# QuantumSavory/LDPCDecoders.jl

Measured on AMD Instinct MI355X. Metric: decoded syndromes/sec (batchdecode!, 50 iters) + achieved HBM GB/s fraction, higher is better.
Workload: dtype f64

## Files before the change

### include/ldpc_mi355x_debug.h

```cpp
#ifndef LDPC_MI355X_DEBUG_H
#define LDPC_MI355X_DEBUG_H

#include "ldpc_mi355x.h"

#ifdef __cplusplus
extern "C" {
#endif

ldpc_status ldpc_debug_team_plan(int64_t nnz, int64_t max_iters, int64_t batch, int32_t cache_mib, int32_t rows_dv,
                                 int32_t out[6]);

ldpc_status ldpc_debug_team_rows(int64_t s, int64_t n, const int64_t *colptr, const int64_t *rowval, int32_t members,
                                 int32_t regs_per_wave, int32_t static_quarters, int32_t *degrees, int32_t *shape,
                                 int32_t *vtab, int32_t *ctab, int32_t *lds_edge, int32_t *reg_edge);

ldpc_status ldpc_debug_team_irr(int64_t s, int64_t n, const int64_t *colptr, const int64_t *rowval, int32_t members,
                                int32_t dc_bucket, int32_t dv_bucket, int32_t *shape, int32_t *ctab2, int32_t *ptab, int32_t *ploc,
                                int32_t *lds_edge, int32_t *posmap);

void *ldpc_debug_process_state(void);
ldpc_status ldpc_debug_adopt_process_state(void *state);

ldpc_status ldpc_debug_div_check(int64_t count, const double *num, const double *den, double *out_core, double *out_ieee);

ldpc_status ldpc_debug_llr_check(int64_t count, const double *odds, double *out_fast, double *out_lib);

#ifdef __cplusplus
}
#endif
#endif
```

### ldpcdecoders.jl_amd/_capi.py

```python
from __future__ import annotations

import ctypes
import os
import subprocess

_HERE = os.path.dirname(os.path.abspath(__file__))
CSRC = os.path.join(_HERE, "csrc")
LIB_PATH = os.environ.get("LDPC_MI355X_LIB") or os.path.join(CSRC, "libldpc_mi355x.so")
EXP_LIB_PATH = os.environ.get("LDPC_MI355X_EXP_LIB") or os.path.join(CSRC, "libldpc_mi355x_exp.so")

LDPC_OK = 0
STATUS_NAMES = {
    0: "LDPC_OK",
    1: "LDPC_ERR_INVALID_ARGUMENT",
    2: "LDPC_ERR_NO_DEVICE",
    3: "LDPC_ERR_HIP",
    4: "LDPC_ERR_OUT_OF_MEMORY",
    5: "LDPC_ERR_UNSUPPORTED",
}

EXPORTED_SYMBOLS = (
    "ldpc_abi_version",
    "ldpc_build_target",
    "ldpc_last_error",
# ... 14 lines not shown
    "ldpc_bp_call_phase_ticks",
    "ldpc_bp_create_multi",
    "ldpc_bp_destroy_multi",
    "ldpc_bp_multi_handle",
    "ldpc_bp_decode_batch_multi",
    "ldpc_bp_decode_batch_multi_bits",
    "ldpc_bp_decode_batch_multi_device",
    "ldpc_bp_multi_last_status",
    "ldpc_bp_multi_get_info",
    "ldpc_osd_create",
    "ldpc_osd_destroy",
    "ldpc_osd_postprocess_batch",
    "ldpc_bpots_create",
    "ldpc_bpots_destroy",
    "ldpc_bpots_kernel",
    "ldpc_bpots_decode_batch",
    "ldpc_bpots_decode_batch_device",
    "ldpc_bitflip_create",
    "ldpc_bitflip_destroy",
    "ldpc_bitflip_kernel",
    "ldpc_bitflip_decode_batch",
    "ldpc_bitflip_decode_batch_device",
)
DEBUG_SYMBOLS = ("ldpc_debug_team_rows", "ldpc_debug_team_plan", "ldpc_debug_div_check", "ldpc_debug_process_state",
                 "ldpc_debug_adopt_process_state", "ldpc_debug_team_irr", "ldpc_debug_llr_check")

MULTI_MAX_DEVICES = 16
EXCHANGE_AUTO, EXCHANGE_COPY, EXCHANGE_RCCL, EXCHANGE_NONE = 0, 1, 2, 3


class LdpcError(RuntimeError):
    def __init__(self, status: int, message: str):
        super().__init__(f"{STATUS_NAMES.get(status, status)}: {message}")
        self.status = status
        self.message = message


class BPInfo(ctypes.Structure):
    _fields_ = [
        ("s", ctypes.c_int64), ("n", ctypes.c_int64), ("nnz", ctypes.c_int64),
        ("max_iters", ctypes.c_int64), ("per", ctypes.c_double),
        ("max_check_degree", ctypes.c_int32), ("max_bit_degree", ctypes.c_int32),
        ("device", ctypes.c_int32), ("tile_syndromes", ctypes.c_int32),
        ("waves_per_tile", ctypes.c_int32), ("resident_tiles", ctypes.c_int32),
        ("workspace_bytes", ctypes.c_int64),
        ("last_kernel", ctypes.c_int32), ("last_team_size", ctypes.c_int32),
        ("last_lds_rows", ctypes.c_int32), ("last_rows_on_chip", ctypes.c_int32), ("reserved_info", ctypes.c_int32 * 2),
# ... 60 lines not shown
    path = EXP_LIB_PATH if experiments else LIB_PATH
    if not os.path.exists(path):
        raise LdpcError(2, f"{path} is not built; run `python -c 'import __graft_entry__ as g; g.build()'` "
                           "or `make -C ldpcdecoders.jl_amd/csrc`. There is no CPU fallback.")
    _one_hip_runtime()
    L = ctypes.CDLL(path)
    vp, i64, i32, f64 = ctypes.c_void_p, ctypes.c_int64, ctypes.c_int32, ctypes.c_double
    L.ldpc_abi_version.restype = i32
    L.ldpc_build_target.restype = ctypes.c_char_p
    L.ldpc_last_error.restype = ctypes.c_char_p
    L.ldpc_device_count.restype = i32
    L.ldpc_trim_memory.restype = i32
    L.ldpc_set_wait_limit_ms.restype = i32
    L.ldpc_set_wait_limit_ms.argtypes = [i64]
    L.ldpc_get_wait_limit_ms.restype = i64
    L.ldpc_debug_team_plan.restype = i32
    L.ldpc_debug_team_plan.argtypes = [i64, i64, i64, i32, i32, ctypes.POINTER(i32 * 6)]
    L.ldpc_debug_div_check.restype = i32
    L.ldpc_debug_div_check.argtypes = [i64, vp, vp, vp, vp]
    L.ldpc_debug_llr_check.restype = i32
    L.ldpc_debug_llr_check.argtypes = [i64, vp, vp, vp]
    L.ldpc_debug_team_irr.restype = i32
    L.ldpc_debug_team_irr.argtypes = [i64, i64, vp, vp, i32, i32, i32, ctypes.POINTER(i32 * 2), vp, vp, vp, vp, vp]
    L.ldpc_debug_team_rows.restype = i32
    L.ldpc_debug_team_rows.argtypes = [i64, i64, vp, vp, i32, i32, i32, ctypes.POINTER(i32 * 2), ctypes.POINTER(i32 * 5), vp, vp, vp, vp]
    L.ldpc_bp_create_multi.restype = i32
    L.ldpc_bp_create_multi.argtypes = [i32, ctypes.POINTER(i32), i32, i64, i64, i64, vp, vp, f64, i64, ctypes.POINTER(BPOptions), ctypes.POINTER(vp)]
    L.ldpc_bp_destroy_multi.restype = i32
    L.ldpc_bp_destroy_multi.argtypes = [vp]
    L.ldpc_bp_multi_handle.restype = vp
    L.ldpc_bp_multi_handle.argtypes = [vp, i32]
    L.ldpc_bp_decode_batch_multi.restype = i32
    L.ldpc_bp_decode_batch_multi.argtypes = [vp, i64, vp, vp, vp, vp, vp]
    L.ldpc_bp_decode_batch_multi_device.restype = i32
    L.ldpc_bp_decode_batch_multi_device.argtypes = [vp, i64, vp, vp, vp, vp, vp, vp]
    L.ldpc_bp_multi_last_status.restype = i32
    L.ldpc_bp_multi_last_status.argtypes = [vp]
    L.ldpc_bp_multi_get_info.restype = i32
    L.ldpc_bp_multi_get_info.argtypes = [vp, ctypes.POINTER(BPMultiInfo)]
    L.ldpc_bp_create.restype = i32
    L.ldpc_bp_create.argtypes = [i64, i64, i64, vp, vp, f64, i64, ctypes.POINTER(BPOptions), ctypes.POINTER(vp)]
    L.ldpc_bp_destroy.restype = i32
    L.ldpc_bp_destroy.argtypes = [vp]
    L.ldpc_bp_get_info.restype = i32
    L.ldpc_bp_get_info.argtypes = [vp, ctypes.POINTER(BPInfo)]
    L.ldpc_bp_decode_batch.restype = i32
# ... 65 lines not shown
```

### ldpcdecoders.jl_amd/csrc/bp_team_kernels.hpp

```cpp
#pragma once
#include "bp_kernels.hpp"

#ifndef LDPC_TEAM_THREADS
#define LDPC_TEAM_THREADS 512
#endif
#ifndef LDPC_TEAM_ROWS_WIDE
#define LDPC_TEAM_ROWS_WIDE 1
#endif
#ifndef LDPC_TEAM_TFORM
#define LDPC_TEAM_TFORM 1
#endif
#ifndef LDPC_TEAM_TEST_DIRECT
#define LDPC_TEAM_TEST_DIRECT 1
#endif
#ifndef LDPC_TEAM_SLEEP
#define LDPC_TEAM_SLEEP 16
#endif

namespace ldpc {

__host__ __device__ constexpr int team_vtab_words(int dv) { return 2 * dv + 1 <= 8 ? 8 : 16; }
__host__ __device__ constexpr bool team_rows_degrees_ok(int dc, int dv) { return dc >= 6 && dc <= 10 && dv >= 3 && dv <= 5; }

template <int DV>
struct TeamVRec {
    int pos[DV], lrow[DV], bit;
};
template <int DV>
__device__ __forceinline__ TeamVRec<DV> team_vrec_load(const int *__restrict__ vt)
{
    static_assert(2 * DV + 1 <= 16, "a position record is at most 16 words");
    typedef int v2i __attribute__((ext_vector_type(2)));
    typedef int v4i __attribute__((ext_vector_type(4)));
    typedef int v8i __attribute__((ext_vector_type(8)));
    constexpr int N = 2 * DV + 1;
    int w[16];
// ... 493 lines not shown
    if (deg == 0) return r;
    return bit_dispatch_flat<1, DV>(Mt, L, loc, deg <= DV ? deg : DV, r);
}

template <int DC, int DV, int THREADS, bool LROWS = false>
constexpr int team_min_waves_per_simd()
{
    if (LROWS && LDPC_TEAM_ROWS_WIDE) return THREADS / 256;
    return min_waves_per_simd<DC, DV, THREADS>() < 4 ? min_waves_per_simd<DC, DV, THREADS>() : 4;
}

template <int DC, int DV, bool WANT_LLR, int THREADS, bool RESUMED, bool LROWS = false, int RR = 0, bool IRR = false>
__global__ void
__launch_bounds__(THREADS, (team_min_waves_per_simd<DC, DV, THREADS, LROWS || IRR>()))
bp_team_kernel(BPParams p, TeamParams tp, const int *__restrict__ row_ptr, const int *__restrict__ edge_bit,
               const int *__restrict__ col_ptr, const int *__restrict__ csc2csr,
               const u64 *__restrict__ synmask, const u64 *__restrict__ nevermask)
{
    static_assert(!(LROWS && RESUMED), "packed tiles are decoded where they lie, all rows in global memory");
    static_assert(RR == 0 || (LROWS && RR == kTeamRegRows), "rows in registers come on top of the rows in LDS");
    static_assert(!IRR || (!LROWS && !RESUMED && RR == 0), "irregular graphs: whole checks in LDS, fresh tiles");
    constexpr int RS = IRR ? 2 : 1;
    constexpr bool kTeamHints = (LDPC_TEAM_LIKELY != 0) && DC <= LDPC_TEAM_LIKELY_DC_MAX;
    constexpr bool TF = LROWS && (LDPC_TEAM_TFORM != 0) && DC <= 8;
    auto rget = [&](const int row) -> double {
        if constexpr (RR > 0) return team_reg_get(row);
        else return 0.0;
    };
    auto rput = [&](const bool on, const int row, const double v) {
        if constexpr (RR > 0) {
            if (on) team_reg_put(row, v);
        }
    };
    extern __shared__ double lds_rows[];
    double *const Lr = lds_rows + (threadIdx.x & 63);
    double *const Ldummy = Lr + (size_t)tp.rows.R * kTile;
    __shared__ int sh_ok;
    __shared__ unsigned int sh_deal[2];
#if !LDPC_TEAM_TEST_DIRECT
    __shared__ u64 sh_mism[THREADS / 64];
#endif
    const int lane = threadIdx.x & 63;
    const int w = __builtin_amdgcn_readfirstlane(threadIdx.x >> 6);
    constexpr int W = THREADS / 64;
    const int s = p.s, n = p.n;
    const double r = p.r;
// ... 178 lines not shown
        const size_t cap_rows = ((size_t)n + 3) & ~(size_t)3;
        unsigned int *const cap32 = (unsigned int *)p.llr + (size_t)tile * cap_rows * kTile;
        double *const cap64 = p.llr + (size_t)tile * cap_rows * kTile;
        auto cap_at = [&](int pos) { return ((size_t)(pos >> 2) * kTile + lane) * 4 + (size_t)(pos & 3); };
        auto capture1 = [&](int pos, double T) {
            if (!cap_on) return;
            if (tp.llr_raw == 4) cap32[cap_at(pos)] = llr_hi32(T);
            else cap64[cap_at(pos)] = T;
        };
        auto capture2 = [&](int pos, double T0, double T1) {
            if (!cap_on) return;
            typedef unsigned int v2u __attribute__((ext_vector_type(2)));
            typedef double v2d __attribute__((ext_vector_type(2)));
            if (tp.llr_raw == 4) *(v2u *)(cap32 + cap_at(pos)) = v2u{llr_hi32(T0), llr_hi32(T1)};
            else *(v2d *)(cap64 + cap_at(pos)) = v2d{T0, T1};
        };
        auto capture4 = [&](int pos, const double (&T)[4]) {
            if (!cap_on) return;
            typedef unsigned int v4u __attribute__((ext_vector_type(4)));
            typedef double v2d __attribute__((ext_vector_type(2)));
            if (tp.llr_raw == 4) *(v4u *)(cap32 + cap_at(pos)) = v4u{llr_hi32(T[0]), llr_hi32(T[1]), llr_hi32(T[2]), llr_hi32(T[3])};
            else { *(v2d *)(cap64 + cap_at(pos)) = v2d{T[0], T[1]}; *(v2d *)(cap64 + cap_at(pos) + 2) = v2d{T[2], T[3]}; }
        };
        auto decide = [&](int pos, int j, double T, bool cap = true) {
            const u64 dec = __ballot(T >= 1.0);
            if (WANT_LLR) {
                if (tp.llr_raw >= 4) { if (cap) capture1(pos, T); }
                else if (tp.llr_raw == 0 && ((active >> lane) & 1ull)) p.llr[((size_t)tile * n + j) * kTile + lane] = llr_of(T, p.llr_exact);
            }
            if (lane == 0) em[j] = dec;
        };
        auto chunk = [&](int c) {
            const int j1 = min(n, (c + 1) * vb);
            int j = c * vb;
            if constexpr (LROWS) {
                constexpr int VT = team_vtab_words(DV);
                if constexpr (kFuseFirst) {
                    if (first) {
                        if (j + 4 == j1) {
                            const int *const vt = csc2csr + (size_t)j * VT;
                            const TeamVRec<DV> A = team_vrec_load<DV>(vt), B = team_vrec_load<DV>(vt + VT), C = team_vrec_load<DV>(vt + 2 * VT),
                                               D = team_vrec_load<DV>(vt + 3 * VT);
                            double T[4];
                            T[0] = bit_update_first<DV, DC, TF>(Mt, Lr, sh_first, syn, lane, A.pos, A.lrow, r, rput);
                            T[1] = bit_update_first<DV, DC, TF>(Mt, Lr, sh_first, syn, lane, B.pos, B.lrow, r, rput);
                            T[2] = bit_update_first<DV, DC, TF>(Mt, Lr, sh_first, syn, lane, C.pos, C.lrow, r, rput);
                            T[3] = bit_update_first<DV, DC, TF>(Mt, Lr, sh_first, syn, lane, D.pos, D.lrow, r, rput);
                            decide(j, A.bit & 0x7fffffff, T[0], false);
                            decide(j + 1, B.bit & 0x7fffffff, T[1], false);
                            decide(j + 2, C.bit & 0x7fffffff, T[2], false);
                            decide(j + 3, D.bit & 0x7fffffff, T[3], false);
                            capture4(j, T);
                            return;
                        }
                        for (; j < j1; ++j) {
                            const TeamVRec<DV> A = team_vrec_load<DV>(csc2csr + (size_t)j * VT);
                            decide(j, A.bit & 0x7fffffff, bit_update_first<DV, DC, TF>(Mt, Lr, sh_first, syn, lane, A.pos, A.lrow, r, rput));
                        }
                        return;
                    }
                }
                auto single = [&](const TeamVRec<DV> &a, const int pa) {
                    if (a.bit >= 0) { decide(pa, a.bit, bit_update_exact_v<DV, TF>(Mt, a.pos, r)); return; }
                    if constexpr (RR > 0) {
                        int lo = a.lrow[0];
#pragma unroll
                        for (int k = 1; k < DV; ++k) lo = min(lo, a.lrow[k]);
                        if (lo <= -2) { decide(pa, a.bit & 0x7fffffff, bit_update_onchip<DV, TF>(Mt, Lr, Ldummy, a.pos, a.lrow, r, rget, rput)); return; }
                    }
                    decide(pa, a.bit & 0x7fffffff, bit_update_mixed<DV, TF>(Mt, Lr, a.pos, a.lrow, r));
                };
                auto two = [&](const TeamVRec<DV> &a, const TeamVRec<DV> &b, const int pa) {
                    int rest = -1;
#pragma unroll
                    for (int k = 1; k < DV; ++k) rest &= a.lrow[k] & b.lrow[k];
                    if ((a.bit | b.bit) >= 0 && tp.pairs) {
                        double T0, T1;
                        bit_update_pair_v<DV, TF>(Mt, a.pos, b.pos, r, T0, T1);
                        decide(pa, a.bit, T0, false);
                        decide(pa + 1, b.bit, T1, false);
                        capture2(pa, T0, T1);
                    } else if (rest == -1 && tp.pairs) {
                        double T0, T1;
                        bit_update_pair_first<DV, TF>(Mt, Lr, a.pos, a.lrow[0], b.pos, b.lrow[0], r, rget, rput, T0, T1);
                        decide(pa, a.bit & 0x7fffffff, T0, false);
                        decide(pa + 1, b.bit & 0x7fffffff, T1, false);
                        capture2(pa, T0, T1);
                    } else {
                        single(a, pa);
                        single(b, pa + 1);
                    }
                };
                int q = j;
                if (LDPC_HOT(q + 4 == j1)) {
                    const int *const vt = csc2csr + (size_t)q * VT;
                    const TeamVRec<DV> A = team_vrec_load<DV>(vt), B = team_vrec_load<DV>(vt + VT), C = team_vrec_load<DV>(vt + 2 * VT),
                                       D = team_vrec_load<DV>(vt + 3 * VT);
                    if (LDPC_HOT(tp.pairs & 2)) {
                        int rest = -1;
#pragma unroll
                        for (int k = 1; k < DV; ++k) rest &= A.lrow[k] & B.lrow[k] & C.lrow[k] & D.lrow[k];
                        if (LDPC_HOT(rest == -1)) {
                            int ps[4][DV];
#pragma unroll
                            for (int k = 0; k < DV; ++k) { ps[0][k] = A.pos[k]; ps[1][k] = B.pos[k]; ps[2][k] = C.pos[k]; ps[3][k] = D.pos[k]; }
                            const int lc[4] = {A.lrow[0], B.lrow[0], C.lrow[0], D.lrow[0]};
                            double T[4];
                            constexpr bool KINDS = LDPC_TEAM_CHUNK_KINDS < 0 ? DV == 3 : LDPC_TEAM_CHUNK_KINDS != 0;
                            const int lmin = min(min(lc[0], lc[1]), min(lc[2], lc[3])), lmax = max(max(lc[0], lc[1]), max(lc[2], lc[3]));
                            if (KINDS && RR > 0 && lmax <= -2) bit_update_multi_first<DV, 4, TF, 2>(Mt, Lr, ps, lc, r, rget, rput, T);
                            else if (KINDS && lmin >= 0) bit_update_multi_first<DV, 4, TF, 1>(Mt, Lr, ps, lc, r, rget, rput, T);
                            else bit_update_multi_first<DV, 4, TF, 0>(Mt, Lr, ps, lc, r, rget, rput, T);
                            decide(q, A.bit & 0x7fffffff, T[0], false);
                            decide(q + 1, B.bit & 0x7fffffff, T[1], false);
                            decide(q + 2, C.bit & 0x7fffffff, T[2], false);
                            decide(q + 3, D.bit & 0x7fffffff, T[3], false);
                            capture4(q, T);
                            return;
                        }
                    }
                    two(A, B, q);
                    two(C, D, q + 2);
                    return;
                }
                for (; q + 1 < j1; q += 2) {
                    const int *const vt = csc2csr + (size_t)q * VT;
                    const TeamVRec<DV> A = team_vrec_load<DV>(vt), B = team_vrec_load<DV>(vt + VT);
                    two(A, B, q);
                }
                for (; q < j1; ++q) single(team_vrec_load<DV>(csc2csr + (size_t)q * VT), q);
                return;
            }
            if constexpr (IRR) {
                for (; j < j1; ++j) {
                    const int c0 = col_ptr[2 * j], bw = col_ptr[2 * j + 1];
                    const int deg = col_ptr[2 * j + 2] - c0;
                    const double T = bw >= 0 ? bit_update<DV>(Mt, csc2csr + c0, deg, r) : bit_update_flat<DV>(Mt, Lr, csc2csr + c0, deg, r);
                    decide(j, bw & 0x7fffffff, T);
                }
// ... 49 lines not shown
        if (lane == 0 && mism) __hip_atomic_fetch_or(&mw[it_t - 1], mism, __ATOMIC_RELAXED, __HIP_MEMORY_SCOPE_AGENT);
#else
        if (lane == 0) sh_mism[w] = mism;
        __syncthreads();
        if (threadIdx.x == 0) {
            u64 part = 0;
#pragma unroll
            for (int q = 0; q < W; ++q) part |= sh_mism[q];
            if (part) __hip_atomic_fetch_or(&mw[it_t - 1], part, __ATOMIC_RELAXED, __HIP_MEMORY_SCOPE_AGENT);
        }
#endif
    };
    auto verdict = [&](const int it_t, const u64 *em_t) {
        const u64 U = uniform64(never | __hip_atomic_load(&mw[it_t - 1], __ATOMIC_RELAXED, __HIP_MEMORY_SCOPE_AGENT));
        const int total = it0 + it_t;
        const u64 newly = active & ~U;
        if ((newly >> lane) & 1ull) { my_iters = total; my_conv = 1; }
        active &= U;
        const u64 spent = __ballot(total >= p.max_iters) & active;
        if ((spent >> lane) & 1ull) { my_iters = total; my_conv = 0; }
        active &= ~spent;
        const u64 stopped = newly | spent;
        if (stopped != 0) {
            for (int j = gw * 64 + lane; j < n; j += GW * 64) fin[j] = (fin[j] & ~stopped) | (em_t[j] & stopped);
        }
        quiet = stopped == 0;
        return total;
    };

    while (active != 0) {
        ++it;
        em = (it & 1) ? em_odd : em_even;
        const u64 t0 = wall_clock64();
        const bool fused = kFuseFirst && it == 1 && !resumed;
        if (!have_check && !fused) check_sweep((it == 1) && !resumed);
        const u64 t1 = wall_clock64();
        if (!(fused && placed) && !team_barrier(ctr, G, rank, ++epoch, tp.fault, tp.ticket, &sh_ok, one_xcd, sh_deal)) return;
        if (!placed) {
            if (threadIdx.x == 0)
                sh_one_xcd = __popc(__hip_atomic_load(xccs, __ATOMIC_RELAXED, __HIP_MEMORY_SCOPE_AGENT)) == 1;
            __syncthreads();
            one_xcd = sh_one_xcd != 0 && !tp.always_release;
            placed = true;
        }
        if (have_check) {
            have_check = false;
            verdict(it - 1, ((it - 1) & 1) ? em_odd : em_even);
// ... 100 lines not shown
```

### ldpcdecoders.jl_amd/csrc/ldpc_mi355x.hip

```cpp
#include "../../include/ldpc_mi355x.h"
#include "../../include/ldpc_mi355x_debug.h"
#define LDPC_AUX_KERNELS 1
#include "bp_kernels.hpp"
#include "bp_lds_kernels.hpp"
#include "bp_node_kernels.hpp"
#include "bp_team_kernels.hpp"
#include "bit_io_kernels.hpp"
#include "pickers.hpp"
#include "host_env.hpp"
#include "host_wait.hpp"

#include <algorithm>
#include <atomic>
#include <chrono>
#include <condition_variable>
#include <cstdio>
#include <cstdlib>
#include <cstring>
#include <memory>
#include <mutex>
#include <new>
#include <string>
#include <thread>
#include <utility>
// ... 384 lines not shown
    int last_rows_on_chip = 0;
    int rows_on_chip = 0;
    size_t ws_budget = 0;
    int blocks_cache[2][17];
    int variant = 0;
    bool node_ok = false;
    bool node_msg_lds = false;
    int node_split_check = 0, node_split_edge = 0;
    int64_t node_max_batch = 0;
    int64_t node_take_max = 0;
    DevBuf node_msg;
    DevBuf team_ws, team_ws_lvl[2];
    std::vector<int> h_csc2csr;
    std::vector<int> h_row_ptr, h_edge_bit, h_col_ptr, h_irr_c2r;
    int irr_G = 0, irr_R = 0, irr_on_chip = 0;
    int irr_dcb = 0;
    DevBuf irr_ctab, irr_ptab, irr_ploc, irr_lds_edge, irr_posmap;
    bool team_rows_on = true;
    int rows_dc = 0, rows_dv = 0;
    int rows_G = 0, rows_R = 0;
    int rows_first_c = 0;
    int rows_regs = 0, rows_static_c = 0, rows_static_v = 0;
    DevBuf rows_ctab, rows_vtab, rows_lds_edge, rows_reg_edge, rows_posmap;
    int team_regs = kTeamRegRows;
    bool team_pre_set = false;
    int team_pre = 2;
    int team_flip = 3;
    int team_static_quarters = 3;
    unsigned int *team_fault = nullptr, *team_fault_dev = nullptr;
    int team_per_cu_want = 2;
    int64_t team_min_rows = 2048;
    bool team_min_rows_set = false;
    bool team_no_margin = false, team_always_release = false, team_coop = false;
    int team_max = 32;
    bool team_max_set = false;
    size_t team_cache = (size_t)240 << 20;
    int team_xcds = 0;
    int team_dynamic = 1;
    int team_pairs = 3;
    int team_ahead_from = 1;
    bool team_ahead_set = false;
    bool llr_exact = false;
    int team_llr_raw = 4;
    bool team_llr_footprint = true;
    int team_ahead = 32;
    DevBuf done_ctr;
// ... 28 lines not shown
    static constexpr int kHistory = 16;
    hipEvent_t ev[kRing][4] = {};
    bool timed[kRing] = {};
    bool two_events[kRing] = {};
    bool ctrl_clean[kRing] = {};
    uint64_t ncalls = 0;
    hipStream_t last_stream = nullptr;
    hipEvent_t last_ev = nullptr;
    DevBuf bits_syn, bits_err;
    hipEvent_t bits_ev[kRing][2] = {};
    bool bits_timed[kRing] = {};
    void *bits_pin[kPipe] = {};
    size_t bits_pin_cap[kPipe] = {};
    int inject_fault = 0;
    unsigned rollcall_ticks = 2000000u;

    bool device_idle = false;
    ~ldpc_bp_decoder()
    {
        const bool stalled = ldpc_detail::device_stalled(device);
        const bool idle = device_idle && !stalled;
        DevBuf *all[] = {&row_ptr, &edge_bit, &col_ptr, &csc2csr, &msg, &ctrl, &synmask, &nevermask,
                         &errmask, &finmask, &llr_t, &st_all, &node_msg, &done_ctr, &team_ws, &team_ws_lvl[0], &team_ws_lvl[1], &cold,
                         &rows_ctab, &rows_vtab, &rows_lds_edge, &rows_reg_edge, &rows_posmap,
                         &irr_ctab, &irr_ptab, &irr_ploc, &irr_lds_edge, &irr_posmap, &bits_syn, &bits_err};
        for (DevBuf *b : all) b->release(idle);
        for (int l = 0; l < 2; ++l)
            for (DevBuf *b : {&lvl_state[l], &lvl_list[l], &lvl_it[l], &lvl_syn[l], &lvl_never[l], &lvl_err[l], &lvl_fin[l], &lvl_llr[l]}) b->release(idle);
        for (DevBuf &b : pipe_dev) b.release(idle);
        if (stalled) return;
        if (pin) (void)hipHostFree(pin);
        if (lat_pin) (void)hipHostFree(lat_pin);
        if (team_fault) (void)hipHostFree(team_fault);
        for (void *&q : pipe_pin)
            if (q) (void)hipHostFree(q);
        for (void *&q : bits_pin)
            if (q) (void)hipHostFree(q);
        for (auto &pair : bits_ev)
            for (hipEvent_t &e : pair)
                if (e) (void)hipEventDestroy(e);
        for (hipStream_t &q : pipe_stream)
            if (q) (void)hipStreamDestroy(q);
        for (auto &row : pipe_ev)
            for (hipEvent_t &e : row)
                if (e) (void)hipEventDestroy(e);
        for (auto &slot : ev)
            for (hipEvent_t &e : slot)
// ... 400 lines not shown
{
    if (!dec) return LDPC_OK;
    DeviceGuard guard;
    (void)hipSetDevice(dec->device);
    const ldpc_status st = ldpc_detail::wait_device(dec->device, "ldpc_bp_destroy (device synchronise)");
    dec->device_idle = st == LDPC_OK;
    delete dec;
    return st;
}

ldpc_status ldpc_bp_get_info(const ldpc_bp_decoder *d, ldpc_bp_info *info)
{
    if (!d || !info) return fail(LDPC_ERR_INVALID_ARGUMENT, "NULL argument");
    std::memset(info, 0, sizeof *info);
    info->s = d->s; info->n = d->n; info->nnz = d->nnz; info->max_iters = d->max_iters; info->per = d->per;
    info->max_check_degree = d->max_cdeg; info->max_bit_degree = d->max_bdeg;
    info->device = d->device; info->tile_syndromes = kTile; info->waves_per_tile = d->last_threads / 64;
    info->resident_tiles = d->last_grid;
    const DevBuf *all[] = {&d->row_ptr, &d->edge_bit, &d->col_ptr, &d->csc2csr, &d->msg, &d->ctrl, &d->synmask,
                           &d->nevermask, &d->errmask, &d->finmask, &d->llr_t, &d->st_all, &d->node_msg, &d->pipe_dev[0], &d->pipe_dev[1], &d->pipe_dev[2],
                           &d->lvl_state[0], &d->lvl_state[1], &d->lvl_list[0], &d->lvl_list[1], &d->lvl_it[0], &d->lvl_it[1],
                           &d->lvl_syn[0], &d->lvl_syn[1], &d->lvl_never[0], &d->lvl_never[1], &d->lvl_err[0], &d->lvl_err[1], &d->lvl_fin[0], &d->lvl_fin[1],
                           &d->lvl_llr[0], &d->lvl_llr[1], &d->team_ws, &d->team_ws_lvl[0], &d->team_ws_lvl[1],
                           &d->rows_ctab, &d->rows_vtab, &d->rows_lds_edge, &d->rows_reg_edge, &d->rows_posmap,
                           &d->irr_ctab, &d->irr_ptab, &d->irr_ploc, &d->irr_lds_edge, &d->irr_posmap, &d->bits_syn, &d->bits_err};
    for (const DevBuf *b : all) info->workspace_bytes += (int64_t)b->cap;
    info->last_kernel = d->last_kernel;
    info->last_team_size = d->last_team;
    info->last_lds_rows = d->last_lds_rows;
    info->last_rows_on_chip = d->last_rows_on_chip;
    return LDPC_OK;
}

}

namespace {
struct ProcessState {
    std::mutex team_mu;
    hipEvent_t team_ev[64] = {};
};
ProcessState g_own_state;
ProcessState *g_ps = &g_own_state;
}
extern "C" void *ldpc_debug_process_state(void) { return g_ps; }
extern "C" ldpc_status ldpc_debug_adopt_process_state(void *state)
{
    if (!state) return fail(LDPC_ERR_INVALID_ARGUMENT, "state is NULL");
// ... 80 lines not shown
    int irr_G = 0, irr_on_chip = 0;
    int wide = 0;
};

static int team_rows_expected(const TeamPlanIn &in, int G)
{
    if (!in.rows_possible && in.irr_possible) return G == in.irr_G ? in.irr_on_chip / std::max(G, 1) : 0;
    return in.rows_possible ? (int)std::min<int64_t>(kTeamRowsMax + in.reg_rows, in.nnz / std::max(in.rows_dv, 1) / std::max(G, 1)) : 0;
}

struct TeamRegPlan {
    int regs_per_wave = 0;
    int static_c = 0, static_v = 0;
    int W = LDPC_TEAM_THREADS / 64;
    bool concentrate = true;
    bool whole_checks = false;
    bool strays_last = true;
};
struct TeamRowTables {
    int R = 0;
    int vt = 0;
    size_t in_lds = 0, in_regs = 0;
    std::vector<int> vtab, ctab, lds_edge, reg_edge;
};
static TeamRegPlan team_reg_plan(int n, int s, int G, int regs_per_wave, int quarters, int dv, int dc)
{
    TeamRegPlan rp;
    rp.whole_checks = dv == 3;
    rp.strays_last = dc <= 9;
    const int W = rp.W;
    const int nch_c = (s + kTeamCheckChunk - 1) / kTeamCheckChunk, nch_v = (n + 3) / 4;
    const int min_c = nch_c / G, min_v = nch_v / G;
    rp.static_c = std::max(W, min_c * quarters / 4 / W * W);
    rp.static_v = std::max(W, min_v * quarters / 4 / W * W);
    if (min_c < 2 * W || min_v < 2 * W || quarters <= 0) { rp.static_c = W; rp.static_v = W; }
    else rp.regs_per_wave = regs_per_wave;
    return rp;
}
static TeamRowTables team_rows_tables(int n, int s, int nnz, int dc, int dv, const std::vector<int> &c2r, int G, const TeamRegPlan &rp)
{
    TeamRowTables out;
    const int vt = team_vtab_words(dv), W = rp.W, RC = rp.regs_per_wave;
    auto check_owner = [&](int i) { return (i / kTeamCheckChunk) % G; };
    auto check_wave = [&](int i) { const int l = (i / kTeamCheckChunk) / G; return (RC > 0 && l < rp.static_c) ? l % W : -1; };
    auto pos_wave = [&](int p) { const int l = (p / 4) / G; return (RC > 0 && l < rp.static_v) ? l % W : -1; };
    std::vector<int> cap((size_t)G, 0), member_of_bit((size_t)n, -1);
// ... 92 lines not shown
            size_t b = 0;
            for (int p : pos_of[(size_t)m]) {
                if (bit[(size_t)p] >= 0) continue;
                if (b >= order.size()) std::abort();
                bit[(size_t)p] = order[b++];
            }
        }
    }
    for (int mw = 0; mw < G * W; ++mw) {
        std::sort(reg_rows[(size_t)mw].begin(), reg_rows[(size_t)mw].end());
        for (int x = 0; x < (int)reg_rows[(size_t)mw].size(); ++x) reg_of[(size_t)reg_rows[(size_t)mw][(size_t)x]] = x;
        out.in_regs += reg_rows[(size_t)mw].size();
    }
    int R = 0;
    for (auto &v : cand) R = std::max(R, (int)v.size());
    R = std::max(R, 1);
    std::vector<int> lds_row_of((size_t)nnz, -1);
    std::vector<int> &lds_edge = out.lds_edge, &reg_edge = out.reg_edge;
    lds_edge.assign((size_t)G * R, -1);
    reg_edge.assign((size_t)G * W * std::max(RC, 1), -1);
    std::vector<int> &vtab = out.vtab, &ctab = out.ctab;
    vtab.assign((size_t)n * vt, 0);
    ctab.assign((size_t)s * 4, 0);
    for (int m = 0; m < G; ++m)
        for (int r = 0; r < (int)cand[(size_t)m].size(); ++r) {
            const int q = cand[(size_t)m][(size_t)r], i = q / dc;
            lds_row_of[(size_t)q] = r;
            lds_edge[(size_t)m * R + r] = q;
            if (ctab[(size_t)4 * i] == 0) ctab[(size_t)4 * i + 1] = r;
            ctab[(size_t)4 * i] |= 1 << (q - dc * i);
        }
    for (int mw = 0; mw < G * W; ++mw)
        for (int x = 0; x < (int)reg_rows[(size_t)mw].size(); ++x) {
            const int q = reg_rows[(size_t)mw][(size_t)x], i = q / dc;
            reg_edge[(size_t)mw * RC + x] = q;
            if (ctab[(size_t)4 * i + 2] == 0) ctab[(size_t)4 * i + 3] = x;
            ctab[(size_t)4 * i + 2] |= 1 << (q - dc * i);
        }
    for (int p = 0; p < n; ++p) {
        const int j = bit[(size_t)p];
        bool any = false;
        for (int k = 0; k < dv; ++k) {
            const int q = c2r[(size_t)dv * j + k];
            vtab[(size_t)p * vt + k] = q;
            const int where = reg_of[(size_t)q] >= 0 ? -2 - reg_of[(size_t)q] : lds_row_of[(size_t)q];
            vtab[(size_t)p * vt + dv + k] = where;
            any = any || where != -1;
        }
        vtab[(size_t)p * vt + 2 * dv] = any ? (j | (int)0x80000000u) : j;
    }
    out.R = R;
    out.vt = vt;
    for (auto &v : cand) out.in_lds += v.size();
    return out;
}

extern "C" ldpc_status ldpc_debug_team_rows(int64_t s, int64_t n, const int64_t *colptr, const int64_t *rowval, int32_t members,
                                            int32_t regs_per_wave, int32_t static_quarters, int32_t *degrees, int32_t *shape,
                                            int32_t *vtab, int32_t *ctab, int32_t *lds_edge, int32_t *reg_edge)
{
    if (!colptr || !rowval || !degrees || !shape || !vtab || !ctab || !lds_edge || !reg_edge) return fail(LDPC_ERR_INVALID_ARGUMENT, "NULL argument");
    if (s <= 0 || n <= 0 || members < 1 || members > kTeamMaxMembers || regs_per_wave < 0 || regs_per_wave > kTeamRegRows ||
        static_quarters < 0 || static_quarters > 4)
        return fail(LDPC_ERR_INVALID_ARGUMENT, "bad dimension");
    const int64_t nnz = colptr[n];
    if (nnz <= 0 || nnz % s != 0 || nnz % n != 0 || nnz >= INT32_MAX) return fail(LDPC_ERR_UNSUPPORTED, "not a regular graph");
    const int dc = (int)(nnz / s), dv = (int)(nnz / n);
    if (!team_rows_degrees_ok(dc, dv)) return fail(LDPC_ERR_UNSUPPORTED, "no rows-in-LDS instantiation for this degree pair");
    std::vector<int> fill((size_t)s, 0), c2r((size_t)nnz);
    for (int64_t j = 0; j < n; ++j) {
        if (colptr[j + 1] - colptr[j] != dv) return fail(LDPC_ERR_UNSUPPORTED, "not a regular graph");
        for (int64_t k = colptr[j]; k < colptr[j + 1]; ++k) {
            const int64_t i = rowval[k];
            if (i < 0 || i >= s || fill[(size_t)i] >= dc) return fail(LDPC_ERR_UNSUPPORTED, "not a regular graph");
            c2r[(size_t)k] = (int)(dc * i + fill[(size_t)i]++);
        }
    }
    const TeamRegPlan rp = team_reg_plan((int)n, (int)s, members, regs_per_wave, static_quarters, dv, dc);
    const TeamRowTables t = team_rows_tables((int)n, (int)s, (int)nnz, dc, dv, c2r, members, rp);
    degrees[0] = dc; degrees[1] = dv;
    shape[0] = t.vt; shape[1] = t.R; shape[2] = rp.static_c; shape[3] = rp.static_v; shape[4] = rp.regs_per_wave;
    std::memcpy(vtab, t.vtab.data(), t.vtab.size() * sizeof(int));
    std::memcpy(ctab, t.ctab.data(), t.ctab.size() * sizeof(int));
    std::memcpy(lds_edge, t.lds_edge.data(), t.lds_edge.size() * sizeof(int));
    std::memcpy(reg_edge, t.reg_edge.data(), t.reg_edge.size() * sizeof(int));
    return LDPC_OK;
}

struct TeamIrrTables {
    int R = 1;
    size_t in_lds = 0;
    std::vector<int> ctab2, ptab, ploc, lds_edge, posmap;
};
static TeamIrrTables team_irr_tables(int n, int s, int nnz, const std::vector<int> &row_ptr, const std::vector<int> &edge_bit,
                                     const std::vector<int> &col_ptr, const std::vector<int> &c2r, int G, int dcb, int dvb)
{
    TeamIrrTables out;
    auto owner = [&](int i) { return (i / kTeamCheckChunk) % G; };
    std::vector<int> room_pos((size_t)G, 0), next_lds((size_t)G, 0), member_of_bit((size_t)n, -1), lds_base((size_t)s, -1);
    for (int p = 0; p < n; ++p) room_pos[(size_t)((p / 4) % G)]++;
    for (int i = 0; i < s; ++i) {
        const int e0 = row_ptr[(size_t)i], deg = row_ptr[(size_t)i + 1] - e0, m = owner(i);
        if (deg <= 0 || deg > dcb || room_pos[(size_t)m] < deg || next_lds[(size_t)m] + deg > kTeamRowsMax) continue;
        bool ok = true;
        for (int k = 0; k < deg && ok; ++k) {
            const int j = edge_bit[(size_t)e0 + k];
            ok = member_of_bit[(size_t)j] < 0 && col_ptr[(size_t)j + 1] - col_ptr[(size_t)j] <= dvb;
        }
// ... 143 lines not shown
    if (e == hipSuccess) e = hipMemcpy(out_lib, dv + 2 * count, bytes, hipMemcpyDeviceToHost);
    (void)hipFree(dv);
    if (e != hipSuccess) { (void)hipGetLastError(); return fail(LDPC_ERR_HIP, std::string("ldpc_debug_llr_check: ") + hipGetErrorString(e)); }
    return LDPC_OK;
}

static ldpc_status team_rows_build(ldpc_bp_decoder *d, int G)
{
    if (d->rows_G == G) return LDPC_OK;
    TeamRegPlan rp = team_reg_plan((int)d->n, (int)d->s, G, d->team_regs, d->team_static_quarters, d->rows_dv, d->rows_dc);
    if (const char *e = exp_env("LDPC_TEAM_CONCENTRATE")) { rp.concentrate = std::atoi(e) != 0; rp.whole_checks = std::atoi(e) == 2; }
    if (const char *e = exp_env("LDPC_TEAM_STRAYS_LAST")) rp.strays_last = std::atoi(e) != 0;
    const TeamRowTables t = team_rows_tables((int)d->n, (int)d->s, (int)d->nnz, d->rows_dc, d->rows_dv, d->h_csc2csr, G, rp);
    auto up = [&](DevBuf &b, const std::vector<int> &v) -> ldpc_status {
        ldpc_status r = b.ensure(std::max<size_t>(v.size() * 4, 4));
        if (r != LDPC_OK) return r;
        if (hipMemcpy(b.p, v.data(), v.size() * 4, hipMemcpyHostToDevice) != hipSuccess) { (void)hipGetLastError(); return fail(LDPC_ERR_HIP, "hipMemcpy of the team row tables failed"); }
        return LDPC_OK;
    };
    ldpc_status st;
    if ((st = ldpc_detail::wait_device(d->device, "team row tables (device synchronise before the tables are replaced)")) != LDPC_OK) return st;
    std::vector<int> posmap((size_t)d->n, 0);
    for (int p = 0; p < (int)d->n; ++p) posmap[(size_t)(t.vtab[(size_t)p * t.vt + 2 * d->rows_dv] & 0x7fffffff)] = p;
    if ((st = up(d->rows_posmap, posmap)) != LDPC_OK) return st;
    if ((st = up(d->rows_ctab, t.ctab)) != LDPC_OK || (st = up(d->rows_vtab, t.vtab)) != LDPC_OK ||
        (st = up(d->rows_lds_edge, t.lds_edge)) != LDPC_OK || (st = up(d->rows_reg_edge, t.reg_edge)) != LDPC_OK)
        return st;
    d->rows_G = G; d->rows_R = t.R; d->rows_on_chip = (int)(t.in_lds + t.in_regs);
    d->rows_regs = rp.regs_per_wave; d->rows_static_c = rp.static_c; d->rows_static_v = rp.static_v;
    {
        const int full = (1 << d->rows_dc) - 1, W = LDPC_TEAM_THREADS / 64;
        int first = rp.static_c;
        for (int m = 0; m < G; ++m) {
            int l = 0;
            for (; l < first; ++l) {
                const int64_t i = (int64_t)kTeamCheckChunk * ((int64_t)l * G + m);
                bool whole = i + kTeamCheckChunk <= d->s;
                for (int q = 0; whole && q < kTeamCheckChunk; ++q)
                    whole = t.ctab[(size_t)4 * (i + q)] == full || t.ctab[(size_t)4 * (i + q) + 2] == full;
                if (!whole) break;
            }
            first = std::min(first, l);
        }
        d->rows_first_c = first / W * W;
    }
    if (exp_env("LDPC_TEAM_DEBUG"))
        std::fprintf(stderr, "[ldpc] team rows: %d members, %d LDS rows each at most, %zu of %d edges in LDS, %zu in registers (%d per wave at most; static chunks %d / %d)\n",
// ... 520 lines not shown
        tp.ahead_from = 2;
        tp.llr_raw = 0;
        return LDPC_OK;
    };
    bool team_ran = team > 1;
    int llr_raw_out = 0;
    const int *llr_posmap = nullptr;
    HIP_TRY(hipEventRecord(ev[1], stream));
    if (team > 1) {
        TeamParams tp{};
        if ((st = team_params(d->team_ws, plan.nteams, ntiles, tp)) != LDPC_OK) return st;
        tp.G = team;
        tp.xcds = plan.xcds;
        tp.scatter = team_scatter ? 1 : 0;
        tp.inject_fault = d->inject_fault;
        tp.errmask_alt = (u64 *)d->errmask.p + std::max<size_t>((size_t)ntiles * n, 1);
        tp.ahead_min = d->team_ahead;
        tp.ahead_from = d->team_ahead_from;
        tp.llr_raw = want_llr ? d->team_llr_raw : 0;
        llr_raw_out = tp.llr_raw == 6 ? 4 : tp.llr_raw;
        if (plan.scatter && !d->team_ahead_set && tp.ahead_min > 0) tp.ahead_min = 1;
        team_kernel_t tk = pick_team_kernel(d->max_cdeg, d->max_bdeg, want_llr);
        size_t team_lds = team_lds_bytes();
        const int *t_col = a_col, *t_c2r = a_c2r, *t_row = a_row;
        if (plan.irr && !team_scatter && team_irr_build(d, team) == LDPC_OK && d->irr_on_chip > 0) {
            team_kernel_t tki = pick_team_kernel_irr(d->irr_dcb, d->max_bdeg, want_llr);
            const size_t need = (size_t)d->irr_R * kTile * sizeof(double);
            int occ_irr = 0;
            if (tki && d->prepare_kernel((const void *)tki, LDPC_TEAM_THREADS, need, &occ_irr) == LDPC_OK && occ_irr >= 1) {
                tk = tki; team_lds = need;
                d->last_lds_rows = d->irr_R; d->last_rows_on_chip = d->irr_on_chip;
                tp.rows.lds_edge = (const int *)d->irr_lds_edge.p;
                tp.rows.R = d->irr_R;
                tp.rows.reg_edge = nullptr; tp.rows.regs = 0;
                tp.rows.static_c = tp.rows.static_v = LDPC_TEAM_THREADS / 64; tp.rows.flip = 0;
                t_row = (const int *)d->irr_ctab.p;
                t_col = (const int *)d->irr_ptab.p;
                t_c2r = (const int *)d->irr_ploc.p;
                llr_posmap = (const int *)d->irr_posmap.p;
            }
        }
        if (plan.rows && team_rows_build(d, team) == LDPC_OK) {
            team_kernel_t tkr = pick_team_kernel_rows(d->rows_dc, d->rows_dv, want_llr, d->rows_regs > 0);
            const size_t need = (size_t)(d->rows_R + (d->rows_regs > 0 ? 1 : 0)) * kTile * sizeof(double);
            int occ_rows = 0;
            if (tkr && d->prepare_kernel((const void *)tkr, LDPC_TEAM_THREADS, need, &occ_rows) == LDPC_OK && occ_rows >= 1) {
                tk = tkr; team_lds = need;
                d->last_lds_rows = d->rows_R; d->last_rows_on_chip = d->rows_on_chip;
                tp.rows.lds_edge = (const int *)d->rows_lds_edge.p;
                tp.rows.R = d->rows_R;
                tp.rows.reg_edge = (const int *)d->rows_reg_edge.p;
                tp.rows.regs = d->rows_regs;
                tp.rows.static_c = d->rows_static_c; tp.rows.static_v = d->rows_static_v; tp.rows.flip = d->team_flip;
                tp.rows.first_c = d->rows_first_c;
                tp.pre = std::min((plan.wide && !d->team_pre_set) ? 8 : d->team_pre, d->rows_first_c / (LDPC_TEAM_THREADS / 64));
                t_col = (const int *)d->rows_ctab.p;
                t_c2r = (const int *)d->rows_vtab.p;
                llr_posmap = (const int *)d->rows_posmap.p;
            }
        }
        const u64 *a_syn = (const u64 *)d->synmask.p, *a_nev = (const u64 *)d->nevermask.p;
        void *args[] = {&p, &tp, &t_row, &a_eb, &t_col, &t_c2r, &a_syn, &a_nev};
        const hipError_t te = launch_team_grid(d, tk, team_grid, args, stream, team_lds);
        if (te != hipSuccess) {
            (void)hipGetLastError();
            d->team_max = 1;
            threads = tile_threads; grid = tile_grid;
            d->last_kernel = 1; d->last_team = 1; d->last_lds_rows = 0; d->last_rows_on_chip = 0; d->last_grid = grid; d->last_threads = threads;
            if ((st = ensure_workspace(d, (size_t)grid * slot_stride_bytes, grid, slot_stride_bytes, stream)) != LDPC_OK) return st;
            p.msg = (double *)d->msg.p;
            kfn = pick_kernel(d->max_cdeg, d->max_bdeg, want_llr, threads);
            team_ran = false;
            llr_raw_out = 0;
            llr_posmap = nullptr;
        }
        if (team_ran && exp_env("LDPC_TEAM_DEBUG")) {
            const int nt = std::min(plan.nteams, ntiles);
            std::vector<unsigned> xm((size_t)nt);
            (void)ldpc_detail::wait_stream(stream, d->device, "LDPC_TEAM_DEBUG (stream synchronise)");
            for (int t = 0; t < nt; ++t)
                (void)hipMemcpy(&xm[(size_t)t], tp.ctl + (size_t)t * kTeamCtlWords + 32, sizeof(unsigned), hipMemcpyDeviceToHost);
            int single = 0;
            for (unsigned v : xm) single += __builtin_popcount(v) == 1;
            std::fprintf(stderr, "[ldpc] team kernel: %d tiles, %d teams x %d workgroups, grid %d; %d teams on one XCD (first masks %x %x %x)\n",
                         ntiles, plan.nteams, team, team_grid, single, xm[0], nt > 1 ? xm[1] : 0u, nt > 2 ? xm[2] : 0u);
// ... 605 lines not shown
```

Before: 94520.

## Store rows-kernel hard decisions by position and remap edges to positions

In the rows-in-LDS team kernel, per-bit decision words are now stored indexed by vertex position rather than bit index, so groups of four or two consecutive decisions are written by adjacent lanes (or one vector store) instead of scattered single-lane stores. The edge-to-bit table passed to the kernel is replaced with an edge-to-position table, and the final mask merge maps position back to bit through the vtab. The aim is to coalesce the decision writes; the cost is an extra indirect gather in the stop path and relaxed atomic stores by default.

```diff
diff --git a/include/ldpc_mi355x_debug.h b/include/ldpc_mi355x_debug.h
--- a/include/ldpc_mi355x_debug.h
+++ b/include/ldpc_mi355x_debug.h
@@ -14,6 +14,10 @@
                                  int32_t regs_per_wave, int32_t static_quarters, int32_t *degrees, int32_t *shape,
                                  int32_t *vtab, int32_t *ctab, int32_t *lds_edge, int32_t *reg_edge);
 
+ldpc_status ldpc_debug_team_rows_pos(int64_t s, int64_t n, const int64_t *colptr, const int64_t *rowval, int32_t members,
+                                     int32_t regs_per_wave, int32_t static_quarters, int32_t *edge_bit, int32_t *edge_pos,
+                                     int32_t *bit_of_pos);
+
 ldpc_status ldpc_debug_team_irr(int64_t s, int64_t n, const int64_t *colptr, const int64_t *rowval, int32_t members,
                                 int32_t dc_bucket, int32_t dv_bucket, int32_t *shape, int32_t *ctab2, int32_t *ptab, int32_t *ploc,
                                 int32_t *lds_edge, int32_t *posmap);
diff --git a/ldpcdecoders.jl_amd/_capi.py b/ldpcdecoders.jl_amd/_capi.py
--- a/ldpcdecoders.jl_amd/_capi.py
+++ b/ldpcdecoders.jl_amd/_capi.py
@@ -60,7 +60,7 @@
     "ldpc_bitflip_decode_batch",
     "ldpc_bitflip_decode_batch_device",
 )
-DEBUG_SYMBOLS = ("ldpc_debug_team_rows", "ldpc_debug_team_plan", "ldpc_debug_div_check", "ldpc_debug_process_state",
+DEBUG_SYMBOLS = ("ldpc_debug_team_rows", "ldpc_debug_team_rows_pos", "ldpc_debug_team_plan", "ldpc_debug_div_check", "ldpc_debug_process_state",
                  "ldpc_debug_adopt_process_state", "ldpc_debug_team_irr", "ldpc_debug_llr_check")
 
 MULTI_MAX_DEVICES = 16
@@ -167,6 +167,8 @@
     L.ldpc_debug_llr_check.argtypes = [i64, vp, vp, vp]
     L.ldpc_debug_team_irr.restype = i32
     L.ldpc_debug_team_irr.argtypes = [i64, i64, vp, vp, i32, i32, i32, ctypes.POINTER(i32 * 2), vp, vp, vp, vp, vp]
+    L.ldpc_debug_team_rows_pos.restype = i32
+    L.ldpc_debug_team_rows_pos.argtypes = [i64, i64, vp, vp, i32, i32, i32, vp, vp, vp]
     L.ldpc_debug_team_rows.restype = i32
     L.ldpc_debug_team_rows.argtypes = [i64, i64, vp, vp, i32, i32, i32, ctypes.POINTER(i32 * 2), ctypes.POINTER(i32 * 5), vp, vp, vp, vp]
     L.ldpc_bp_create_multi.restype = i32
diff --git a/ldpcdecoders.jl_amd/csrc/bp_team_kernels.hpp b/ldpcdecoders.jl_amd/csrc/bp_team_kernels.hpp
--- a/ldpcdecoders.jl_amd/csrc/bp_team_kernels.hpp
+++ b/ldpcdecoders.jl_amd/csrc/bp_team_kernels.hpp
@@ -12,6 +12,15 @@
 #endif
 #ifndef LDPC_TEAM_TEST_DIRECT
 #define LDPC_TEAM_TEST_DIRECT 1
+#endif
+#ifndef LDPC_TEAM_NO_DEC_STORE
+#define LDPC_TEAM_NO_DEC_STORE 0
+#endif
+#ifndef LDPC_TEAM_DEC_BY_POS
+#define LDPC_TEAM_DEC_BY_POS 1
+#endif
+#ifndef LDPC_TEAM_DEC_STORE_KIND
+#define LDPC_TEAM_DEC_STORE_KIND 0
 #endif
 #ifndef LDPC_TEAM_SLEEP
 #define LDPC_TEAM_SLEEP 16
@@ -551,6 +560,7 @@
     static_assert(!IRR || (!LROWS && !RESUMED && RR == 0), "irregular graphs: whole checks in LDS, fresh tiles");
     constexpr int RS = IRR ? 2 : 1;
     constexpr bool kTeamHints = (LDPC_TEAM_LIKELY != 0) && DC <= LDPC_TEAM_LIKELY_DC_MAX;
+    constexpr bool kDecByPos = LROWS && (LDPC_TEAM_DEC_BY_POS != 0);
     constexpr bool TF = LROWS && (LDPC_TEAM_TFORM != 0) && DC <= 8;
     auto rget = [&](const int row) -> double {
         if constexpr (RR > 0) return team_reg_get(row);
@@ -775,13 +785,52 @@
             if (tp.llr_raw == 4) *(v4u *)(cap32 + cap_at(pos)) = v4u{llr_hi32(T[0]), llr_hi32(T[1]), llr_hi32(T[2]), llr_hi32(T[3])};
             else { *(v2d *)(cap64 + cap_at(pos)) = v2d{T[0], T[1]}; *(v2d *)(cap64 + cap_at(pos) + 2) = v2d{T[2], T[3]}; }
         };
-        auto decide = [&](int pos, int j, double T, bool cap = true) {
+        auto put_word = [&](u64 *at, u64 dec) {
+#if !LDPC_TEAM_NO_DEC_STORE
+            if constexpr (kDecByPos && LDPC_TEAM_DEC_STORE_KIND == 0) __hip_atomic_store(at, dec, __ATOMIC_RELAXED, __HIP_MEMORY_SCOPE_AGENT);
+            else *at = dec;
+#else
+            asm volatile("" :: "v"(dec));
+#endif
+        };
+#if LDPC_TEAM_DEC_STORE_KIND == 2
+        typedef u64 v2w __attribute__((ext_vector_type(2), aligned(8)));
+#endif
+        auto put2 = [&](int pos, u64 d0, u64 d1) {
+#if LDPC_TEAM_DEC_STORE_KIND == 2 && !LDPC_TEAM_NO_DEC_STORE
+            if (lane == 0) *(v2w *)(em + pos) = v2w{d0, d1};
+#else
+            const u64 dec = (lane & 1) ? d1 : d0;
+            if (lane < 2) put_word(em + pos + lane, dec);
+#endif
+        };
+        auto put4 = [&](int pos, u64 d0, u64 d1, u64 d2, u64 d3) {
+#if LDPC_TEAM_DEC_STORE_KIND == 2 && !LDPC_TEAM_NO_DEC_STORE
+            if (lane == 0) { *(v2w *)(em + pos) = v2w{d0, d1}; *(v2w *)(em + pos + 2) = v2w{d2, d3}; }
+#else
+            const u64 lo = (lane & 1) ? d1 : d0, hi = (lane & 1) ? d3 : d2;
+            const u64 dec = (lane & 2) ? hi : lo;
+            if (lane < 4) put_word(em + pos + lane, dec);
+#endif
+        };
+        auto decide = [&](int pos, int j, double T, bool cap = true, bool store = true) -> u64 {
             const u64 dec = __ballot(T >= 1.0);
             if (WANT_LLR) {
                 if (tp.llr_raw >= 4) { if (cap) capture1(pos, T); }
                 else if (tp.llr_raw == 0 && ((active >> lane) & 1ull)) p.llr[((size_t)tile * n + j) * kTile + lane] = llr_of(T, p.llr_exact);
             }
-            if (lane == 0) em[j] = dec;
+            if (store && lane == 0) put_word(em + (kDecByPos ? pos : j), dec);
+            return dec;
+        };
+        auto decide4 = [&](int pos, const int (&bits)[4], const double (&T)[4]) {
+            u64 d[4];
+#pragma unroll
+            for (int b = 0; b < 4; ++b) d[b] = decide(pos + b, bits[b] & 0x7fffffff, T[b], false, !kDecByPos);
+            if constexpr (kDecByPos) put4(pos, d[0], d[1], d[2], d[3]);
+        };
+        auto decide_pair = [&](int pos, int bit0, int bit1, double T0, double T1) {
+            const u64 d0 = decide(pos, bit0 & 0x7fffffff, T0, false, !kDecByPos), d1 = decide(pos + 1, bit1 & 0x7fffffff, T1, false, !kDecByPos);
+            if constexpr (kDecByPos) put2(pos, d0, d1);
         };
         auto chunk = [&](int c) {
             const int j1 = min(n, (c + 1) * vb);
@@ -799,10 +848,8 @@
                             T[1] = bit_update_first<DV, DC, TF>(Mt, Lr, sh_first, syn, lane, B.pos, B.lrow, r, rput);
                             T[2] = bit_update_first<DV, DC, TF>(Mt, Lr, sh_first, syn, lane, C.pos, C.lrow, r, rput);
                             T[3] = bit_update_first<DV, DC, TF>(Mt, Lr, sh_first, syn, lane, D.pos, D.lrow, r, rput);
-                            decide(j, A.bit & 0x7fffffff, T[0], false);
-                            decide(j + 1, B.bit & 0x7fffffff, T[1], false);
-                            decide(j + 2, C.bit & 0x7fffffff, T[2], false);
-                            decide(j + 3, D.bit & 0x7fffffff, T[3], false);
+                            const int bits[4] = {A.bit, B.bit, C.bit, D.bit};
+                            decide4(j, bits, T);
                             capture4(j, T);
                             return;
                         }
@@ -830,14 +877,12 @@
                     if ((a.bit | b.bit) >= 0 && tp.pairs) {
                         double T0, T1;
                         bit_update_pair_v<DV, TF>(Mt, a.pos, b.pos, r, T0, T1);
-                        decide(pa, a.bit, T0, false);
-                        decide(pa + 1, b.bit, T1, false);
+                        decide_pair(pa, a.bit, b.bit, T0, T1);
                         capture2(pa, T0, T1);
                     } else if (rest == -1 && tp.pairs) {
                         double T0, T1;
                         bit_update_pair_first<DV, TF>(Mt, Lr, a.pos, a.lrow[0], b.pos, b.lrow[0], r, rget, rput, T0, T1);
-                        decide(pa, a.bit & 0x7fffffff, T0, false);
-                        decide(pa + 1, b.bit & 0x7fffffff, T1, false);
+                        decide_pair(pa, a.bit, b.bit, T0, T1);
                         capture2(pa, T0, T1);
                     } else {
                         single(a, pa);
@@ -864,10 +909,8 @@
                             if (KINDS && RR > 0 && lmax <= -2) bit_update_multi_first<DV, 4, TF, 2>(Mt, Lr, ps, lc, r, rget, rput, T);
                             else if (KINDS && lmin >= 0) bit_update_multi_first<DV, 4, TF, 1>(Mt, Lr, ps, lc, r, rget, rput, T);
                             else bit_update_multi_first<DV, 4, TF, 0>(Mt, Lr, ps, lc, r, rget, rput, T);
-                            decide(q, A.bit & 0x7fffffff, T[0], false);
-                            decide(q + 1, B.bit & 0x7fffffff, T[1], false);
-                            decide(q + 2, C.bit & 0x7fffffff, T[2], false);
-                            decide(q + 3, D.bit & 0x7fffffff, T[3], false);
+                            const int bits[4] = {A.bit, B.bit, C.bit, D.bit};
+                            decide4(q, bits, T);
                             capture4(q, T);
                             return;
                         }
@@ -963,7 +1006,15 @@
         active &= ~spent;
         const u64 stopped = newly | spent;
         if (stopped != 0) {
-            for (int j = gw * 64 + lane; j < n; j += GW * 64) fin[j] = (fin[j] & ~stopped) | (em_t[j] & stopped);
+            if constexpr (kDecByPos) {
+                constexpr int VT = team_vtab_words(DV);
+                for (int j = gw * 64 + lane; j < n; j += GW * 64) {
+                    const int b = csc2csr[(size_t)j * VT + 2 * DV] & 0x7fffffff;
+                    fin[b] = (fin[b] & ~stopped) | (em_t[j] & stopped);
+                }
+            } else {
+                for (int j = gw * 64 + lane; j < n; j += GW * 64) fin[j] = (fin[j] & ~stopped) | (em_t[j] & stopped);
+            }
         }
         quiet = stopped == 0;
         return total;
diff --git a/ldpcdecoders.jl_amd/csrc/ldpc_mi355x.hip b/ldpcdecoders.jl_amd/csrc/ldpc_mi355x.hip
--- a/ldpcdecoders.jl_amd/csrc/ldpc_mi355x.hip
+++ b/ldpcdecoders.jl_amd/csrc/ldpc_mi355x.hip
@@ -430,6 +430,7 @@
     int rows_first_c = 0;
     int rows_regs = 0, rows_static_c = 0, rows_static_v = 0;
     DevBuf rows_ctab, rows_vtab, rows_lds_edge, rows_reg_edge, rows_posmap;
+    DevBuf rows_edge_pos;
     int team_regs = kTeamRegRows;
     bool team_pre_set = false;
     int team_pre = 2;
@@ -504,7 +505,7 @@
         const bool idle = device_idle && !stalled;
         DevBuf *all[] = {&row_ptr, &edge_bit, &col_ptr, &csc2csr, &msg, &ctrl, &synmask, &nevermask,
                          &errmask, &finmask, &llr_t, &st_all, &node_msg, &done_ctr, &team_ws, &team_ws_lvl[0], &team_ws_lvl[1], &cold,
-                         &rows_ctab, &rows_vtab, &rows_lds_edge, &rows_reg_edge, &rows_posmap,
+                         &rows_ctab, &rows_vtab, &rows_lds_edge, &rows_reg_edge, &rows_posmap, &rows_edge_pos,
                          &irr_ctab, &irr_ptab, &irr_ploc, &irr_lds_edge, &irr_posmap, &bits_syn, &bits_err};
         for (DevBuf *b : all) b->release(idle);
         for (int l = 0; l < 2; ++l)
@@ -951,7 +952,7 @@
                            &d->lvl_state[0], &d->lvl_state[1], &d->lvl_list[0], &d->lvl_list[1], &d->lvl_it[0], &d->lvl_it[1],
                            &d->lvl_syn[0], &d->lvl_syn[1], &d->lvl_never[0], &d->lvl_never[1], &d->lvl_err[0], &d->lvl_err[1], &d->lvl_fin[0], &d->lvl_fin[1],
                            &d->lvl_llr[0], &d->lvl_llr[1], &d->team_ws, &d->team_ws_lvl[0], &d->team_ws_lvl[1],
-                           &d->rows_ctab, &d->rows_vtab, &d->rows_lds_edge, &d->rows_reg_edge, &d->rows_posmap,
+                           &d->rows_ctab, &d->rows_vtab, &d->rows_lds_edge, &d->rows_reg_edge, &d->rows_posmap, &d->rows_edge_pos,
                            &d->irr_ctab, &d->irr_ptab, &d->irr_ploc, &d->irr_lds_edge, &d->irr_posmap, &d->bits_syn, &d->bits_err};
     for (const DevBuf *b : all) info->workspace_bytes += (int64_t)b->cap;
     info->last_kernel = d->last_kernel;
@@ -1078,6 +1079,7 @@
     int vt = 0;
     size_t in_lds = 0, in_regs = 0;
     std::vector<int> vtab, ctab, lds_edge, reg_edge;
+    std::vector<int> edge_pos;
 };
 static TeamRegPlan team_reg_plan(int n, int s, int G, int regs_per_wave, int quarters, int dv, int dc)
 {
@@ -1216,6 +1218,7 @@
     std::vector<int> &vtab = out.vtab, &ctab = out.ctab;
     vtab.assign((size_t)n * vt, 0);
     ctab.assign((size_t)s * 4, 0);
+    out.edge_pos.assign((size_t)nnz, 0);
     for (int m = 0; m < G; ++m)
         for (int r = 0; r < (int)cand[(size_t)m].size(); ++r) {
             const int q = cand[(size_t)m][(size_t)r], i = q / dc;
@@ -1237,6 +1240,7 @@
         for (int k = 0; k < dv; ++k) {
             const int q = c2r[(size_t)dv * j + k];
             vtab[(size_t)p * vt + k] = q;
+            out.edge_pos[(size_t)q] = p;
             const int where = reg_of[(size_t)q] >= 0 ? -2 - reg_of[(size_t)q] : lds_row_of[(size_t)q];
             vtab[(size_t)p * vt + dv + k] = where;
             any = any || where != -1;
@@ -1278,6 +1282,35 @@
     std::memcpy(ctab, t.ctab.data(), t.ctab.size() * sizeof(int));
     std::memcpy(lds_edge, t.lds_edge.data(), t.lds_edge.size() * sizeof(int));
     std::memcpy(reg_edge, t.reg_edge.data(), t.reg_edge.size() * sizeof(int));
+    return LDPC_OK;
+}
+
+extern "C" ldpc_status ldpc_debug_team_rows_pos(int64_t s, int64_t n, const int64_t *colptr, const int64_t *rowval, int32_t members,
+                                                int32_t regs_per_wave, int32_t static_quarters, int32_t *edge_bit, int32_t *edge_pos,
+                                                int32_t *bit_of_pos)
+{
+    if (!colptr || !rowval || !edge_bit || !edge_pos || !bit_of_pos) return fail(LDPC_ERR_INVALID_ARGUMENT, "NULL argument");
+    if (s <= 0 || n <= 0 || members < 1 || members > kTeamMaxMembers || regs_per_wave < 0 || regs_per_wave > kTeamRegRows ||
+        static_quarters < 0 || static_quarters > 4)
+        return fail(LDPC_ERR_INVALID_ARGUMENT, "bad dimension");
+    const int64_t nnz = colptr[n];
+    if (nnz <= 0 || nnz % s != 0 || nnz % n != 0 || nnz >= INT32_MAX) return fail(LDPC_ERR_UNSUPPORTED, "not a regular graph");
+    const int dc = (int)(nnz / s), dv = (int)(nnz / n);
+    if (!team_rows_degrees_ok(dc, dv)) return fail(LDPC_ERR_UNSUPPORTED, "no rows-in-LDS instantiation for this degree pair");
+    std::vector<int> fill((size_t)s, 0), c2r((size_t)nnz);
+    for (int64_t j = 0; j < n; ++j) {
+        if (colptr[j + 1] - colptr[j] != dv) return fail(LDPC_ERR_UNSUPPORTED, "not a regular graph");
+        for (int64_t k = colptr[j]; k < colptr[j + 1]; ++k) {
+            const int64_t i = rowval[k];
+            if (i < 0 || i >= s || fill[(size_t)i] >= dc) return fail(LDPC_ERR_UNSUPPORTED, "not a regular graph");
+            c2r[(size_t)k] = (int)(dc * i + fill[(size_t)i]);
+            edge_bit[(size_t)(dc * i + fill[(size_t)i]++)] = (int)j;
+        }
+    }
+    const TeamRegPlan rp = team_reg_plan((int)n, (int)s, members, regs_per_wave, static_quarters, dv, dc);
+    const TeamRowTables t = team_rows_tables((int)n, (int)s, (int)nnz, dc, dv, c2r, members, rp);
+    std::memcpy(edge_pos, t.edge_pos.data(), t.edge_pos.size() * sizeof(int));
+    for (int64_t p = 0; p < n; ++p) bit_of_pos[p] = t.vtab[(size_t)p * t.vt + 2 * dv] & 0x7fffffff;
     return LDPC_OK;
 }
 
@@ -1467,7 +1500,7 @@
     if ((st = ldpc_detail::wait_device(d->device, "team row tables (device synchronise before the tables are replaced)")) != LDPC_OK) return st;
     std::vector<int> posmap((size_t)d->n, 0);
     for (int p = 0; p < (int)d->n; ++p) posmap[(size_t)(t.vtab[(size_t)p * t.vt + 2 * d->rows_dv] & 0x7fffffff)] = p;
-    if ((st = up(d->rows_posmap, posmap)) != LDPC_OK) return st;
+    if ((st = up(d->rows_posmap, posmap)) != LDPC_OK || (st = up(d->rows_edge_pos, t.edge_pos)) != LDPC_OK) return st;
     if ((st = up(d->rows_ctab, t.ctab)) != LDPC_OK || (st = up(d->rows_vtab, t.vtab)) != LDPC_OK ||
         (st = up(d->rows_lds_edge, t.lds_edge)) != LDPC_OK || (st = up(d->rows_reg_edge, t.reg_edge)) != LDPC_OK)
         return st;
@@ -2034,7 +2067,7 @@
         if (plan.scatter && !d->team_ahead_set && tp.ahead_min > 0) tp.ahead_min = 1;
         team_kernel_t tk = pick_team_kernel(d->max_cdeg, d->max_bdeg, want_llr);
         size_t team_lds = team_lds_bytes();
-        const int *t_col = a_col, *t_c2r = a_c2r, *t_row = a_row;
+        const int *t_col = a_col, *t_c2r = a_c2r, *t_row = a_row, *t_eb = a_eb;
         if (plan.irr && !team_scatter && team_irr_build(d, team) == LDPC_OK && d->irr_on_chip > 0) {
             team_kernel_t tki = pick_team_kernel_irr(d->irr_dcb, d->max_bdeg, want_llr);
             const size_t need = (size_t)d->irr_R * kTile * sizeof(double);
@@ -2069,10 +2102,11 @@
                 t_col = (const int *)d->rows_ctab.p;
                 t_c2r = (const int *)d->rows_vtab.p;
                 llr_posmap = (const int *)d->rows_posmap.p;
+                if (LDPC_TEAM_DEC_BY_POS) t_eb = (const int *)d->rows_edge_pos.p;
             }
         }
         const u64 *a_syn = (const u64 *)d->synmask.p, *a_nev = (const u64 *)d->nevermask.p;
-        void *args[] = {&p, &tp, &t_row, &a_eb, &t_col, &t_c2r, &a_syn, &a_nev};
+        void *args[] = {&p, &tp, &t_row, &t_eb, &t_col, &t_c2r, &a_syn, &a_nev};
         const hipError_t te = launch_team_grid(d, tk, team_grid, args, stream, team_lds);
         if (te != hipSuccess) {
             (void)hipGetLastError();
```

Result: no change. 94890 (median of 6 runs) (+0.4%).
